# hal0zer0/openwurli

Measured on AMD Instinct MI355X. Metric: audio samples/s, 64-voice full chain (x real-time @48 kHz = value / 48000), higher is better.
Workload: dtype f64

## Files before the change

openwurli_amd/csrc/host/host_pool.inc:

```
namespace {
void trem_groups_changed(ow_pool* p) {
    HIP_OK(hipMemcpyAsync(p->d_lead, p->h_lead, sizeof(uint32_t) * p->I, hipMemcpyHostToDevice, p->stream));
    p->lead_list_valid = false;
    p->split_e0 = p->split_ne = -1;
}
void trem_split_at_range(ow_pool* p, int e0, int ne) {
    const uint32_t I = (uint32_t)p->I, lo = (uint32_t)e0, hi = (uint32_t)(e0 + ne);
    if (ne >= (int)I || (p->split_e0 == e0 && p->split_ne == ne)) return;
    const uint32_t NONE = 0xFFFFFFFFu;
    bool straddle = false;
    std::fill(p->grp_in.begin(), p->grp_in.end(), NONE);
    std::fill(p->grp_out.begin(), p->grp_out.end(), NONE);
    for (uint32_t e = 0; e < I; ++e) {
        const uint32_t x = p->h_lead[e];
        uint32_t& slot = (e >= lo && e < hi) ? p->grp_in[x] : p->grp_out[x];
        if (slot == NONE) slot = e;
    }
    size_t n_copy = 0;
    for (uint32_t x = 0; x < I; ++x) {
        if (p->grp_in[x] == NONE || p->grp_out[x] == NONE) continue;
        straddle = true;
        const bool x_inside = x >= lo && x < hi;
        const uint32_t fresh = x_inside ? p->grp_out[x] : p->grp_in[x];
        p->h_copy[n_copy] = x; p->h_copy[I + n_copy] = fresh; ++n_copy;
// ... 390 lines not shown
    return own_osc || hit ? p->rb_cur : -1;
}

struct Packed { bool any_dirty = false; size_t n_ops = 0; uint32_t n_act = 0; bool any_main = false, any_steal = false; };
static Packed pack_args_and_ops(ow_pool* p, const Block& b) {
    const int e0 = b.e0, ne = b.ne;
    Packed r;
    const bool untouched = b.whole && !__atomic_load_n(&p->dirty_any, __ATOMIC_RELAXED) && !p->args_stale && p->any_cache_valid;
    if (b.whole) __atomic_store_n(&p->dirty_any, (uint8_t)0, __ATOMIC_RELAXED);
    size_t n_dirty = 0;
    if (!untouched) for (int k = 0; k < ne; ++k) n_dirty += p->dirty[e0 + k];
    size_t T = (n_dirty >= 4096) ? std::min<size_t>(effective_cpus(), 32) : 1;
    const int per = (int)((ne + T - 1) / T);
    size_t cnt[OW_MAX_SLICES + 1] = {0};
    uint8_t dirty_t[OW_MAX_SLICES] = {0};
    auto count_slice = [&](size_t t) {
        size_t c = 0; uint8_t d = 0;
        const int k1 = std::min(ne, (int)(t + 1) * per);
        for (int k = (int)t * per; k < k1; ++k) {
            if (!p->dirty[e0 + k]) continue;
            d = 1;
            c += p->engines[e0 + k]->ops.size();
        }
        cnt[t + 1] = c; dirty_t[t] = d;
    };
    if (!untouched) Workers::get().each(T, count_slice);
    for (size_t t = 0; t < T; ++t) { r.any_dirty = r.any_dirty || dirty_t[t]; cnt[t + 1] += cnt[t]; }
    r.n_ops = cnt[T];
    ensure_ops_capacity(p, r.n_ops);
    if (r.any_dirty || p->args_stale) {
        auto pack_slice = [&](size_t t) {
            size_t op_pos = cnt[t];
            const int k1 = std::min(ne, (int)(t + 1) * per);
            for (int k = (int)t * per; k < k1; ++k) {
                OwEngineArgs& a = p->h_args[e0 + k];
                if (!p->dirty[e0 + k]) {
                    if (a.op_count || a.set_flags) { a.op_count = 0; a.set_flags = 0; }
                    continue;
                }
                ow_engine* en = p->engines[e0 + k].get();
                a.main_mask = en->vm->main_mask; a.steal_mask = en->vm->steal_mask;
                a.noise_on = en->noise_on ? 1u : 0u; a.thermal_gain = en->thermal_gain;
                a.pa_flags = en->rail_sag ? 1u : 0u;
                a.op_begin = (uint32_t)op_pos;
                a.op_count = (uint32_t)en->ops.size();
                if (!en->ops.empty()) std::memcpy(p->h_ops + op_pos, en->ops.data(), sizeof(OwOp) * en->ops.size());
                if (const uint32_t nd = en->vm->n_dev_ops) {
                    if (!en->ops.empty()) {
                        const uint32_t room = OW_VM_OPS_MAX - nd, nh = (uint32_t)std::min<size_t>(en->ops.size(), room);
                        if (nh < en->ops.size()) {
                            const uint64_t lost = g_ops_dropped.fetch_add(en->ops.size() - nh) + (en->ops.size() - nh);
                            if (lost == en->ops.size() - nh)
                                std::fprintf(stderr, "openwurli-hip: engine %zu: %zu queued slot ops do not fit behind a device-side MIDI burst (OW_MIDI_APPLY_EARLY=0) and are dropped\n",
                                             (size_t)(e0 + k), en->ops.size() - nh);
                        }
                        std::lock_guard<std::mutex> lk(p->op_tails_mu);
                        p->op_tails.push_back({(uint32_t)op_pos, (uint32_t)((e0 + k) * OW_VM_OPS_MAX) + nd, nh});
                        a.op_count = nd + nh;
                    } else a.op_count = nd;
                    a.op_begin = 0x80000000u | (uint32_t)((e0 + k) * OW_VM_OPS_MAX);
                    en->vm->n_dev_ops = 0;
                    if (!p->vm_host_dirty) p->vm_host_dirty = 1;
                }
                op_pos += en->ops.size();
                if (!en->ops.empty()) { en->ops.clear(); __atomic_fetch_sub(&p->host_ops_any, 1u, __ATOMIC_RELAXED); }
                a.set_flags = 0;
                if (en->depth.pending) { a.set_flags |= 1u; a.depth_target = en->depth.pending_value; en->depth.pending = false; }
                if (en->spk.pending)   { a.set_flags |= 2u; a.spk_target = en->spk.pending_value;     en->spk.pending = false; }
                if (en->volume.pending){ a.set_flags |= 4u; a.vol_target = en->volume.pending_value;  en->volume.pending = false; }
                p->dirty[e0 + k] = 0;
            }
        };
        Workers::get().each(T, pack_slice);
    }
    r.any_main = p->any_main_c; r.any_steal = p->any_steal_c;
    if (!untouched) {
        const size_t TA = ne >= 16384 ? std::min<size_t>(effective_cpus(), 32) : 1;
        const int per_a = (int)((ne + TA - 1) / TA);
        uint32_t act_n[OW_MAX_SLICES] = {0};
        uint8_t any_m[OW_MAX_SLICES] = {0}, any_s[OW_MAX_SLICES] = {0};
        auto scan_slice = [&](size_t t) {
            const int k0 = (int)t * per_a, k1 = std::min(ne, (int)(t + 1) * per_a);
            uint32_t n = 0; uint8_t m = 0, sl = 0;
            uint32_t* dst = p->h_op_engines + k0;
            for (int k = k0; k < k1; ++k) {
                const OwEngineArgs& a = p->h_args[e0 + k];
                m |= a.main_mask != 0; sl |= a.steal_mask != 0;
                if (a.op_count) dst[n++] = (uint32_t)(e0 + k);
            }
            act_n[t] = n; any_m[t] = m; any_s[t] = sl;
        };
        Workers::get().each(TA, scan_slice);
        r.any_main = false; r.any_steal = false;
        for (size_t t = 0; t < TA; ++t) {
            r.any_main |= any_m[t] != 0; r.any_steal |= any_s[t] != 0;
            if (act_n[t] && r.n_act != (uint32_t)(t * per_a)) std::memmove(p->h_op_engines + r.n_act, p->h_op_engines + t * per_a, sizeof(uint32_t) * act_n[t]);
            r.n_act += act_n[t];
        }
        if (b.whole) { p->any_main_c = r.any_main; p->any_steal_c = r.any_steal; p->any_cache_valid = true; }
    }
    return r;
}

static void upload_and_apply_ops(ow_pool* p, const Block& b, const Packed& pk) {
    const int e0 = b.e0, ne = b.ne;
    hipStream_t st = p->stream;
    if (pk.any_dirty || p->args_stale) {
        HIP_OK(hipMemcpyAsync(p->d_args + e0, p->h_args + e0, sizeof(OwEngineArgs) * ne, hipMemcpyHostToDevice, st));
        p->args_stale = pk.any_dirty;
    }
    HIP_OK(hipMemsetAsync(p->d_eout + e0, 0, sizeof(OwEngineOut) * ne, st));
    if (p->profiling) HIP_OK(hipEventRecord(p->ev[0], st));
    if (pk.n_ops || p->dev_ops_pending) {
        if (pk.n_ops) HIP_OK(hipMemcpyAsync(p->d_ops, p->h_ops, sizeof(OwOp) * pk.n_ops, hipMemcpyHostToDevice, st));
        for (const ow_pool::OpTail& t : p->op_tails)
            HIP_OK(hipMemcpyAsync(p->d_ops_fix + t.dst, p->d_ops + t.src, sizeof(OwOp) * t.n, hipMemcpyDeviceToDevice, st));
        p->op_tails.clear();
        if (pk.n_act) {
            HIP_OK(hipMemcpyAsync(p->d_op_engines, p->h_op_engines, sizeof(uint32_t) * pk.n_act, hipMemcpyHostToDevice, st));
            owdev::k_apply_ops<<<dim3(pk.n_act), dim3(64), 0, st>>>(p->dK, p->d_nt, p->d_vrec, p->d_args, p->d_ops, p->d_op_engines, p->d_ops_fix);
        }
        if (b.whole) p->dev_ops_pending = false;
    }
    if (p->profiling) HIP_OK(hipEventRecord(p->ev[1], st));
}

static bool launch_voices(ow_pool* p, const Block& b) {
    const int I = (int)p->I, L = b.L, Lcap = (int)p->Lcap;
    hipStream_t s = p->stream;
    const unsigned bs = p->vl_steady.n_blocks, bg = p->vl_general.n_blocks, bt = p->vl_steal.n_blocks, ba = p->vl_attack.n_blocks;
    if (ba) owdev::k_voice_steady<false, 1><<<dim3(ba), dim3(64), 0, s>>>(p->dK, p->d_vrec, p->vl_attack.d, p->d_sum, p->d_eout, I, L, Lcap, nullptr);
    if (bs) {
        if (p->sw.voice_skew && p->skew_next)
            owdev::k_voice_steady<true><<<dim3(bs), dim3(64), 0, s>>>(p->dK, p->d_vrec, p->vl_steady.d, p->d_sum, p->d_eout, I, L, Lcap, p->d_skew_seen);
        else
            owdev::k_voice_steady<false><<<dim3(bs), dim3(64), 0, s>>>(p->dK, p->d_vrec, p->vl_steady.d, p->d_sum, p->d_eout, I, L, Lcap, p->d_skew_seen);
    }
    if (bg) {
        const bool rel = p->sw.voice_release && !p->sw.force_general;
        if (rel) owdev::k_voice_steady<false, 3><<<dim3(bg), dim3(64), 0, s>>>(p->dK, p->d_vrec, p->vl_general.d, p->d_sum, p->d_eout, I, L, Lcap, nullptr);
        owdev::k_voice<<<dim3(bg), dim3(64), 0, s>>>(p->dK, p->d_vrec, p->vl_general.d, p->d_sum, p->d_eout, I, L, Lcap, rel ? 4 : 0);
    }
    if (bt) {
        if (p->sw.voice_steal) owdev::k_voice_steady<false, 2><<<dim3(bt), dim3(64), 0, s>>>(p->dK, p->d_vrec, p->vl_steal.d, p->d_sum, p->d_eout, I, L, Lcap, nullptr);
        owdev::k_voice<<<dim3(bt), dim3(64), 0, s>>>(p->dK, p->d_vrec, p->vl_steal.d, p->d_sum, p->d_eout, I, L, Lcap, p->sw.voice_steal ? 5 : 1);
    }
    return bs != 0;
}

static bool launch_chain(ow_pool* p, const Block& b, ChainKernel kernel) {
    const int I = (int)p->I, L = b.L, Lcap = (int)p->Lcap, e0 = b.e0, ne = b.ne;
    hipStream_t s = p->stream;
    const owdev::OwTremSrc& tsrc = b.tsrc;
    const dim3 per8((ne + 7) / 8), per32((ne + 31) / 32), per64((ne + 63) / 64);
    const int generic = p->sw.mel_generic ? 1 : 0;
    switch (kernel) {
    case CHAIN_NONE: break;
    case CHAIN_ROW_OS_8: owdev::k_chain_row<true, 8><<<per8, dim3(320), 0, s>>>(p->dK, p->d_cs, p->d_args, p->d_eout, p->d_sum, tsrc, p->d_pre, p->d_out, I, L, Lcap, L, e0, ne); break;
    case CHAIN_ROW_OS_16: owdev::k_chain_row<true, 16><<<per8, dim3(320), 0, s>>>(p->dK, p->d_cs, p->d_args, p->d_eout, p->d_sum, tsrc, p->d_pre, p->d_out, I, L, Lcap, L, e0, ne); break;
    case CHAIN_ROW_8: owdev::k_chain_row<false, 8><<<per8, dim3(320), 0, s>>>(p->dK, p->d_cs, p->d_args, p->d_eout, p->d_sum, tsrc, p->d_pre, p->d_out, I, L, Lcap, L, e0, ne); break;
    case CHAIN_ROW_16: owdev::k_chain_row<false, 16><<<per8, dim3(320), 0, s>>>(p->dK, p->d_cs, p->d_args, p->d_eout, p->d_sum, tsrc, p->d_pre, p->d_out, I, L, Lcap, L, e0, ne); break;
    case CHAIN_FUSED_OS: owdev::k_chain_fused<true><<<per8, dim3(128), 0, s>>>(p->dK, p->d_cs, p->d_args, p->d_eout, p->d_sum, tsrc, p->d_pre, p->d_out, I, L, Lcap, L, e0, ne); break;
    case CHAIN_FUSED: owdev::k_chain_fused<false><<<per8, dim3(128), 0, s>>>(p->dK, p->d_cs, p->d_args, p->d_eout, p->d_sum, tsrc, p->d_pre, p->d_out, I, L, Lcap, L, e0, ne); break;
    case CHAIN_STREAM:
        owdev::k_chain_stream<<<per32, dim3(64), 0, s>>>(p->dK, p->d_cs, p->d_args, p->d_eout, p->d_sum, tsrc, p->d_pre, p->d_out, I, L, Lcap, L, e0, ne, b.out_direct, b.out_stride);
        return b.out_direct != nullptr;
    case PREAMP_MEL_ENG:
        owdev::k_preamp_mel_eng<<<per64, dim3(64), 0, s>>>(p->dK, p->d_cs, p->d_mel_settled, p->d_args, p->d_eout, p->d_sum, tsrc, p->d_pre, p->d_noise, I, L, Lcap, e0, ne, generic, p->d_mel_lu, p->mel_lu_ld);
        break;
    case PREAMP_MEL_COL:
        owdev::k_preamp_mel_col<<<per32, dim3(64), 0, s>>>(p->dK, p->d_cs, p->d_mel_settled, p->d_args, p->d_eout, p->d_sum, tsrc, p->d_pre, p->d_noise, I, L, Lcap, e0, ne, generic, p->d_mel_lu, p->mel_lu_ld);
        break;
    case PREAMP_MEL_LIT:
        owdev::k_preamp_mel_lit<<<per32, dim3(64), 0, s>>>(p->dK, p->d_cs, p->d_mel_settled, p->d_args, p->d_eout, p->d_sum, tsrc, p->d_pre, p->d_noise, I, L, Lcap, e0, ne, generic, p->d_mel_lu);
        break;
    case PREAMP_MEL: owdev::k_preamp_mel<<<per32, dim3(64), 0, s>>>(p->dK, p->d_cs, p->d_mel_settled, p->d_args, p->d_eout, p->d_sum, tsrc, p->d_pre, p->d_noise, I, L, Lcap, e0, ne); break;
    case PREAMP_WIDE: owdev::k_preamp_wide<<<per8, dim3(64), 0, s>>>(p->dK, p->d_cs, p->d_args, p->d_eout, p->d_sum, tsrc, p->d_pre, I, L, Lcap, e0, ne); break;
    case PREAMP_PAIR: owdev::k_preamp_pair<<<per64, dim3(64), 0, s>>>(p->dK, p->d_cs, p->d_args, p->d_eout, p->d_sum, tsrc, p->d_pre, I, L, Lcap, e0, ne); break;
    case PREAMP_LANE: owdev::k_preamp<<<per32, dim3(64), 0, s>>>(p->dK, p->d_cs, p->d_args, p->d_eout, p->d_sum, tsrc, p->d_pre, I, L, Lcap, e0, ne); break;
    }
    return false;
}

static bool launch_output_stage(ow_pool* p, const Block& b, PostKernel kernel) {
    const int I = (int)p->I, L = b.L, e0 = b.e0, ne = b.ne;
    hipStream_t s = p->stream;
    switch (kernel) {
    case POST_NONE: return false;
    case POST_MPA: {
        const bool ordered = p->sw.pa_sort != 0 && ne > power_amp_resident_engines(p);
        if (ordered) {
            const uint32_t total = (uint32_t)b.n_os;
            HIP_OK(hipMemsetAsync(p->d_pa_hist, 0, sizeof(uint32_t) * PA_ORDER_CLASSES, s));
            owdev::k_pa_order_hist<<<dim3((ne + 255) / 256), dim3(256), 0, s>>>(p->d_pa_demand, e0, ne, total, p->d_pa_hist);
            owdev::k_pa_order_scan<<<dim3(1), dim3(PA_ORDER_CLASSES), 0, s>>>(p->d_pa_hist);
            owdev::k_pa_order_scatter<<<dim3((ne + 255) / 256), dim3(256), 0, s>>>(p->d_pa_demand, e0, ne, total, p->d_pa_hist, p->d_pa_order);
        }
        owdev::k_post_mpa<<<dim3((ne + PA_EPB - 1) / PA_EPB), dim3(PA_WPB * 64), 0, s>>>(p->dK, p->dPa, p->d_pa_settled, p->d_cs, p->d_pa, p->d_args, p->d_eout, p->d_pre, p->d_out,
                                                                                     p->d_pa_tap, I, L, L, e0, ne, ordered ? p->d_pa_order : nullptr, p->d_pa_demand);
        return false;
    }
    case POST_PAIR: owdev::k_post<false, true><<<dim3((ne + 63) / 64), dim3(64), 0, s>>>(p->dK, p->d_cs, p->d_args, p->d_eout, p->d_pre, p->d_out, I, L, L, e0, ne, b.out_direct, b.out_stride); break;
    case POST_OS: owdev::k_post<true><<<dim3((ne + 31) / 32), dim3(64), 0, s>>>(p->dK, p->d_cs, p->d_args, p->d_eout, p->d_pre, p->d_out, I, L, L, e0, ne, b.out_direct, b.out_stride); break;
    case POST_BASE: owdev::k_post<false><<<dim3((ne + 63) / 64), dim3(64), 0, s>>>(p->dK, p->d_cs, p->d_args, p->d_eout, p->d_pre, p->d_out, I, L, L, e0, ne, b.out_direct, b.out_stride); break;
    }
    return b.out_direct != nullptr;
}

static void deliver_rows(ow_pool* p, const Block& b) {
    const float* src = p->d_out + (size_t)b.e0 * b.len;
    if (b.out_stride == b.len) HIP_OK(hipMemcpyAsync(b.out_host, src, sizeof(float) * b.len * (size_t)b.ne, hipMemcpyDeviceToHost, p->stream));
    else HIP_OK(hipMemcpy2DAsync(b.out_host, b.out_stride * sizeof(float), src, b.len * sizeof(float), b.len * sizeof(float), (size_t)b.ne, hipMemcpyDeviceToHost, p->stream));
}

static void finish_block(ow_pool* p, const Block& b, bool steady_launched) {
    const int e0 = b.e0, ne = b.ne, n_os = b.n_os;
    hipStream_t st = p->stream;
    if (b.chain && p->traj) {
        if (b.whole) p->trem_clock += n_os;
        else {
            for (int k = 0; k < ne; ++k) if (p->h_birth[e0 + k] != OW_OFF_TRAJ) { p->h_birth[e0 + k] -= n_os; p->min_birth = std::min(p->min_birth, p->h_birth[e0 + k]); }
            owdev::k_trem_birth_shift<<<dim3((ne + 255) / 256), dim3(256), 0, st>>>(p->d_birth, e0, ne, -(long long)n_os);
        }
    }
    p->last_n_os = n_os;
    HIP_OK(hipGetLastError());
    if (steady_launched) {
        HIP_OK(hipMemcpyAsync(p->h_skew_seen, p->d_skew_seen, sizeof(uint32_t), hipMemcpyDeviceToHost, st));
        p->skew_pending = true;
    }
    if (eout_attention(p, ne)) {
        if (p->attn_resync) {
            std::memcpy(p->h_prev_tr, p->transient.data(), p->I);
            HIP_OK(hipMemcpyAsync(p->d_prev_tr, p->h_prev_tr, p->I, hipMemcpyHostToDevice, st));
            p->attn_resync = false;
        }
        owdev::k_eout_attention<<<dim3((ne + 255) / 256), dim3(256), 0, st>>>(p->d_eout, p->d_args, p->d_prev_tr, e0, ne, p->d_attn);
        HIP_OK(hipGetLastError());
        HIP_OK(hipMemcpyAsync(p->h_attn, p->d_attn, sizeof(uint64_t) * ((ne + 63) / 64), hipMemcpyDeviceToHost, st));
        p->attn_pending = true;
    } else {
        HIP_OK(hipMemcpyAsync(p->h_eout + e0, p->d_eout + e0, sizeof(OwEngineOut) * ne, hipMemcpyDeviceToHost, st));
        p->attn_pending = false;
    }
}

void render_range(ow_pool* p, int e0, int ne, size_t len, bool with_voices, float* out_host = nullptr, size_t out_stride = 0) {
    if (len > p->Lcap) { HIP_OK(hipStreamSynchronize(p->stream)); alloc_stream_buffers(p, len); }
    p->out_ld = len;
    hipStream_t st = p->stream;
    auto profile_mark = [&](int i) { if (p->profiling) HIP_OK(hipEventRecord(p->ev_stage[i], st)); };
    vm_wait_download(p);
    Block b;
    b.e0 = e0; b.ne = ne; b.len = len; b.L = (int)len; b.n_os = b.L * (p->hc.oversample ? 2 : 1);
    b.whole = e0 == 0 && ne == (int)p->I;
    b.chain = !p->voices_only;
    b.out_host = out_host; b.out_stride = out_stride;
    b.tsrc = owdev::OwTremSrc{nullptr, p->d_lead, nullptr, p->d_birth};
    const hipEvent_t traj_ready = b.chain && p->traj ? traj_cover_block(p, b) : nullptr;
    const int trem_half = trem_block(p, b);
    const Packed pk = pack_args_and_ops(p, b);
    upload_and_apply_ops(p, b, pk);
    const bool voices = with_voices && (pk.any_main || pk.any_steal);
    if (voices) {
        if (!p->lists_valid || pk.any_dirty || p->lists_e0 != e0 || p->lists_ne != ne) build_voice_lists(p, e0, ne);
        p->lists_valid = !pk.any_dirty;
        if (p->vl_steady.n_blocks) HIP_OK(hipMemsetAsync(p->d_skew_seen, 0, sizeof(uint32_t), st));
    }
    if (out_host && p->sw.out_direct != 0 && out_stride >= len && ne > 0)
        b.out_direct = (float*)host_block_device_ptr(out_host, sizeof(float) * ((size_t)(ne - 1) * out_stride + len));
    profile_mark(0);
    const bool steady_launched = voices && launch_voices(p, b);
    profile_mark(1);
    if (trem_half >= 0) HIP_OK(hipStreamWaitEvent(st, p->ev_trem[trem_half], 0));
    if (traj_ready) HIP_OK(hipStreamWaitEvent(st, traj_ready, 0));
    profile_mark(2);
    const ChainKernel chain = !b.chain ? CHAIN_NONE
        : choose_chain(p->sw, (int)p->hc.preamp_kind, p->power_amp_kind, p->hc.oversample != 0, p->hc.ml_sparse_ok != 0, ne, b.L, b.out_direct != nullptr);
    bool delivered = launch_chain(p, b, chain);
    profile_mark(3);
    delivered |= launch_output_stage(p, b, choose_post(p->sw, p->power_amp_kind, p->hc.oversample != 0, ne, chain));
    profile_mark(4);
    if (out_host && ne > 0 && !delivered) deliver_rows(p, b);
    finish_block(p, b, steady_launched);
}

void engine_steal_countdown(ow_engine* en, uint32_t l32) {
    OwVm& v = *en->vm;
    if (!v.steal_mask) return;
    vm_host_changed(en);
    for (uint64_t m = v.steal_mask; m; m &= m - 1) {
        const int s = __builtin_ctzll(m);
        v.steal_fade[s] = v.steal_fade[s] > l32 ? v.steal_fade[s] - l32 : 0u;
        if (v.steal_fade[s] == 0) { v.has_steal &= ~(1ull << s); en->sync_masks(s); }
    }
}
void engine_post_render(ow_engine* en, uint32_t l32, const OwEngineOut& o, bool steal_counted = false) {
    OwVm& v = *en->vm;
    vm_host_changed(en);
    if (!steal_counted) engine_steal_countdown(en, l32);
    if (o.sum_nonfinite) {
        en->nan_guard_fires += 1;
        for (int s = 0; s < OW_MAX_VOICES; ++s) {
            const uint64_t b = 1ull << s;
            if ((o.bad_main >> s) & 1ull) { en->set_state(s, OW_VOICE_FREE); v.has_voice &= ~b; }
            if ((o.bad_steal >> s) & 1ull) { v.has_steal &= ~b; v.steal_fade[s] = 0; }
            en->sync_masks(s);
        }
    }
    if (o.out_nonfinite) en->output_nan_resets += 1;
    for (uint64_t m = o.silent_mask & v.main_mask; m; m &= m - 1) {
        const int s = __builtin_ctzll(m);
        if (en->state_of(s) != OW_VOICE_FREE && ((v.has_voice >> s) & 1ull)) { en->set_state(s, OW_VOICE_FREE); v.has_voice &= ~(1ull << s); en->sync_masks(s); }
    }
}

void engine_guard_second_pass_result(ow_engine* en, const OwEngineOut& o) {
    OwVm& v = *en->vm;
    vm_host_changed(en);
    for (int s = 0; s < OW_MAX_VOICES; ++s) {
        const uint64_t b = 1ull << s;
        bool touched = false;
        if ((o.bad_main >> s) & 1ull) { en->set_state(s, OW_VOICE_FREE); v.has_voice &= ~b; touched = true; }
        if ((o.bad_steal >> s) & 1ull) { v.has_steal &= ~b; v.steal_fade[s] = 0; touched = true; }
        if (touched) en->sync_masks(s);
    }
    for (uint64_t m = o.silent_mask & v.main_mask; m; m &= m - 1) {
        const int s = __builtin_ctzll(m);
        if (en->state_of(s) != OW_VOICE_FREE && ((v.has_voice >> s) & 1ull)) { en->set_state(s, OW_VOICE_FREE); v.has_voice &= ~(1ull << s); en->sync_masks(s); }
    }
}
void guard_second_pass(ow_pool* p, const uint32_t* engs, size_t n_eng, size_t len) {
    hipStream_t st = p->stream;
    uint32_t nm = 0, ns = 0;
    for (size_t i = 0; i < n_eng; ++i) {
        const ow_engine* en = p->engines[engs[i]].get();
        auto put = [&](uint32_t* a, uint32_t& n, uint64_t mask) {
            if (!mask) return;
            for (uint64_t m = mask; m; m &= m - 1) a[n++] = (engs[i] << 6) | (uint32_t)__builtin_ctzll(m);
            while (n & 63u) a[n++] = 0xFFFFFFFFu;
        };
        put(p->vl_general.h, nm, en->vm->main_mask);
        put(p->vl_steal.h, ns, en->vm->steal_mask);
    }
    p->lists_valid = false;
    p->vl_general.sig_valid = false; p->vl_steal.sig_valid = false;
    const unsigned nb = (unsigned)((n_eng + 255) / 256);
    HIP_OK(hipMemcpyAsync(p->d_op_engines, engs, sizeof(uint32_t) * n_eng, hipMemcpyHostToDevice, st));
    owdev::k_eout_clear_list<<<dim3(nb), dim3(256), 0, st>>>(p->d_eout, p->d_op_engines, (int)n_eng);
    const int I = (int)p->I, L = (int)len, Lcap = (int)p->Lcap;
    if (nm) {
        HIP_OK(hipMemcpyAsync(p->vl_general.d, p->vl_general.h, sizeof(uint32_t) * nm, hipMemcpyHostToDevice, st));
        owdev::k_voice<<<dim3(nm / 64), dim3(64), 0, st>>>(p->dK, p->d_vrec, p->vl_general.d, p->d_sum, p->d_eout, I, L, Lcap, 2);
    }
    if (ns) {
// ... 283 lines not shown
```

openwurli_amd/csrc/ow_kernels.h:

```cpp
#pragma once
#include "ow_vm.h"
#include "ow_chain_dev.h"

namespace owdev {

#define OW_DATA_DECL __device__ const
#define OW_GEN_DATA_REINCLUDE
#include "../../data/ow_gen_data.h"
#undef OW_GEN_DATA_REINCLUDE
#undef OW_DATA_DECL

struct OwEngineOut {
    uint64_t silent_mask;
    uint64_t bad_main;
    uint64_t bad_steal;
    uint32_t sum_nonfinite;
    uint32_t out_nonfinite;
    uint32_t transient;
    uint32_t pad;
};

__device__ inline void mlp_raw_scalar(double in0, double in1, double raw[11]) {
    double h1[16], h2[16];
    for (int i = 0; i < 16; ++i) {
        double sum = MLP_B1[i];
        sum += MLP_W1[i][0] * in0;
        sum += MLP_W1[i][1] * in1;
        h1[i] = sum > 0.0 ? sum : 0.0;
    }
    for (int i = 0; i < 16; ++i) {
        double sum = MLP_B2[i];
        for (int j = 0; j < 16; ++j) sum += MLP_W2[i][j] * h1[j];
        h2[i] = sum > 0.0 ? sum : 0.0;
    }
    for (int i = 0; i < 11; ++i) {
        double sum = MLP_B3[i];
        for (int j = 0; j < 16; ++j) sum += MLP_W3[i][j] * h2[j];
        raw[i] = sum * MLP_TARGET_STDS[i] + MLP_TARGET_MEANS[i];
    }
}

#ifndef OW_APPLY_OPS_ATTR
#define OW_APPLY_OPS_ATTR __attribute__((amdgpu_waves_per_eu(2, 2)))
#endif
__device__ inline void mlp_raw_mfma(double* __restrict__ h, double in0, double in1, double raw[11]);

__global__ __launch_bounds__(64) OW_APPLY_OPS_ATTR void k_apply_ops(const OwConsts* __restrict__ K, const double* __restrict__ nt, double* __restrict__ vrec,
                                                  const OwEngineArgs* __restrict__ args, const OwOp* __restrict__ ops_packed,
                                                  const uint32_t* __restrict__ engines, const OwOp* __restrict__ ops_fixed = nullptr,
                                                  const OwVm* __restrict__ vm = nullptr, int e_base = 0) {
    __shared__ double h[64 * 17];
    const int e = vm ? e_base + (int)blockIdx.x : (int)engines[blockIdx.x];
    const int lane = threadIdx.x;
    OwEngineArgs a;
    if (vm) { a.op_count = vm[e].n_dev_ops; a.op_begin = 0x80000000u | (uint32_t)(e * OW_VM_OPS_MAX); }
    else a = args[e];
    if (a.op_count == 0) return;
    const OwOp* __restrict__ ops = (a.op_begin & 0x80000000u) ? ops_fixed : ops_packed;
    a.op_begin &= 0x7FFFFFFFu;
    double* main_rec = vrec + ((size_t)e * 2 + 0) * OW_VREC_DOUBLES + lane;
    double* steal_rec = vrec + ((size_t)e * 2 + 1) * OW_VREC_DOUBLES + lane;
    constexpr int OPS_TILES = 8;
    uint64_t mine[OPS_TILES];
    const bool tiled = a.op_count <= 64u * OPS_TILES;
    if (tiled) {
#pragma unroll
        for (int t = 0; t < OPS_TILES; ++t) {
            mine[t] = 0ull;
            if ((uint32_t)t * 64u < a.op_count) {
                const uint32_t idx = (uint32_t)t * 64u + (uint32_t)lane;
                const int sl = idx < a.op_count ? (int)ops[a.op_begin + idx].slot : -1;
                for (int v = 0; v < 64; ++v) {
                    const uint64_t m = __ballot(sl == v);
                    if (lane == v) mine[t] = m;
                }
            }
        }
    }
    uint32_t cursor = 0;
    for (;;) {
        asm volatile("" : "+v"(main_rec), "+v"(steal_rec));
        OwOp op;
        op.type = 0;
        if (tiled) {
            bool got = false;
#pragma unroll
            for (int t = 0; t < OPS_TILES; ++t) {
                if (!got && mine[t]) {
                    const int b = __builtin_ctzll(mine[t]);
                    mine[t] &= mine[t] - 1ull;
                    op = ops[a.op_begin + (uint32_t)t * 64u + (uint32_t)b];
                    got = true;
                }
            }
        } else {
            while (cursor < a.op_count) {
                const OwOp cand = ops[a.op_begin + cursor];
                ++cursor;
                if (cand.slot == lane) { op = cand; break; }
            }
        }
        if (!__any(op.type != 0)) break;
        const bool is_on = op.type == OP_NOTE_ON;
        if (__any(is_on)) {
            const double midi = is_on ? (double)op.note : 60.0;
            const double in0 = clampd((midi - 21.0) / (108.0 - 21.0), 0.0, 1.0);
            const double in1 = is_on ? clampd(op.velocity, 0.0, 1.0) : 0.0;
            double raw[11];
            mlp_raw_mfma(h, in0, in1, raw);
            if (is_on) {
                const MlpOut corr = mlp_finish((int)op.note, raw, op.mlp != 0);
                note_on_lane(main_rec, nt, K, (int)op.note, op.velocity, op.seed, corr);
            }
        }
        if (op.type == OP_DAMPER) {
            start_damper_lane(main_rec, K);
        } else if (op.type == OP_SET_DS) {
            main_rec[VF_DS * 64] = op.velocity;
        } else if (op.type == OP_MOVE_STEAL) {
            constexpr int CP = 16;
            for (int f0 = 0; f0 < VF_COUNT; f0 += CP) {
                double t[CP];
#pragma unroll
                for (int k = 0; k < CP; ++k) t[k] = f0 + k < VF_COUNT ? main_rec[(f0 + k) * 64] : 0.0;
#pragma unroll
                for (int k = 0; k < CP; ++k) if (f0 + k < VF_COUNT) steal_rec[(f0 + k) * 64] = t[k];
            }
            steal_rec[VF_STEAL * 64] = bitsd((uint64_t)op.seed | ((uint64_t)op.seed << 32));
        }
    }
}

#ifndef OW_VOICE_GENERAL_ATTR
#define OW_VOICE_GENERAL_ATTR __attribute__((amdgpu_waves_per_eu(2, 2)))
#endif
#define OW_VCHUNK 24
#define OW_NO_VOICE 0xFFFFFFFFu

struct VoiceLanes {
    int e, slot;
    bool active;
    uint64_t seg_end;
    int nvalid;
};
OW_DEV VoiceLanes voice_lanes(const uint32_t* __restrict__ entries, int* __restrict__ eng_l) {
    const int lane = threadIdx.x;
    const uint32_t ent = entries[(size_t)blockIdx.x * 64 + lane];
    VoiceLanes w;
    w.active = ent != OW_NO_VOICE;
    w.e = w.active ? (int)(ent >> 6) : -1;
    w.slot = (int)(ent & 63u);
    eng_l[lane] = w.e;
    const int e_next = __shfl_down(w.e, 1);
    w.seg_end = __ballot(w.active && (lane == 63 || e_next != w.e));
    w.nvalid = __popcll(__ballot(w.active));
// ... 812 lines not shown
        rbuf[(size_t)i * I + e] = trem_cell_r(t, P, K, M + z);
    }
    trem_store(t, P, cs, I, e);
}
__global__ __launch_bounds__(64) void k_tremolo(const OwConsts* __restrict__ K, double* __restrict__ cs, double* __restrict__ rbuf, int I, int n_os,
                                                const uint32_t* __restrict__ leaders, int n_lead) {
    __shared__ TremMats M;
    __shared__ TremPark P;
    tremolo_body(K, cs, rbuf, I, n_os, leaders, n_lead, &M, &P);
}
__global__ __launch_bounds__(64) void k_tremolo_lfo(const OwConsts* __restrict__ K, double* __restrict__ cs, double* __restrict__ rbuf, int I, long long n_os,
                                                    const uint32_t* __restrict__ leaders, int n_lead, long long n_extra) {
    const int idx = blockIdx.x * 64 + threadIdx.x;
    if (idx >= n_lead) return;
    const int e = (int)leaders[idx];
    double phase = CSF(CS_T_V), env = CSF(CS_T_ENV), r_ldr = CSF(CS_T_RLDR);
    const double inc = K->lfo_phase_inc, two_pi = 2.0 * 3.14159265358979323846264338327950288;
    const long long n = n_os + n_extra * idx;
    for (long long i = 0; i < n; ++i) {
        const double lfo = sin(phase);
        phase += inc;
        if (phase >= two_pi) phase -= two_pi;
        const double led = lfo > 0.0 ? lfo : 0.0;
        const double coeff = led > env ? K->ldr_attack : K->ldr_release;
        env = led + coeff * (env - led);
        const double drive = clampd(env, 0.0, 1.0);
        if (drive < 1e-6) r_ldr = 1000000.0;
        else r_ldr = exp(K->ln_r_max + K->ln_min_minus_max * pow(drive, 0.9));
        if (rbuf) rbuf[(size_t)i * I + e] = r_ldr;
    }
    CSF(CS_T_V) = phase; CSF(CS_T_ENV) = env; CSF(CS_T_RLDR) = r_ldr;
}

#define OW_PCHUNK 64
__global__ __launch_bounds__(64) void k_preamp(const OwConsts* __restrict__ K, double* __restrict__ cs, const OwEngineArgs* __restrict__ args,
                                               const OwEngineOut* __restrict__ eout, const double* __restrict__ sum, const OwTremSrc tsrc,
                                               double* __restrict__ pre, int I, int L, int Lcap, int e0, int ne) {
    __shared__ double tile[32 * (OW_PCHUNK + 1)];
    const int lane = threadIdx.x;
    const int el = lane & 31, role = lane >> 5;
    const int eb = e0 + blockIdx.x * 32;
    const int e = eb + el;
    const bool valid = e < e0 + ne;
    const int ec = valid ? e : (e0 + ne - 1);
    const int osr = K->oversample ? 2 : 1;

    DkSt st;
    double ua[3], ub[3];
    double r_ldr, g_ldr, g_prev;
    Smoother sd;
    {
        const int e = ec;
        smoother_load(sd, cs, I, e, CS_SM_DEPTH);
        if (args[e].set_flags & 1u) sd.retarget(args[e].depth_target, K->ramp_samples);
        dk_load(st, cs, I, e, role ? CS_P_SHADOW : CS_P_MAIN);
        for (int i = 0; i < 3; ++i) { ua[i] = CSF(CS_OS_UA + i); ub[i] = CSF(CS_OS_UB + i); }
        r_ldr = CSF(CS_P_RLDR); g_ldr = CSF(CS_P_GLDR); g_prev = CSF(CS_P_GPREV);
        const uint64_t fl = dbits(CSF(CS_FLAGS));
        if (fl & 1ull) {
            dk_dc_reset(K, r_ldr, st);
            g_ldr = 1.0 / r_ldr; g_prev = g_ldr;
            for (int i = 0; i < 3; ++i) { ua[i] = 0.0; ub[i] = 0.0; }
        }
    }
    uint32_t nan_resets = 0;
    double sh_depth = __longlong_as_double(0x7FF8000000000000LL), sh_top = 0.0, sh_lower = 0.0;
    int rowflag = 0;
    {
        const int er = eb + el;
        if (er < e0 + ne && !eout[er].sum_nonfinite) rowflag = (args[er].main_mask ? 1 : 0) | (args[er].steal_mask ? 2 : 0);
    }
    const int e_last = e0 + ne - 1;
    const TremCol tcol = trem_col(tsrc, I, ec);
    double rn[2];
    rn[0] = trem_col_at(tcol, 0u);
    rn[1] = osr == 2 ? trem_col_at(tcol, 1u) : 0.0;
    for (int base = 0; base < L; base += OW_PCHUNK) {
        const int cn = min(OW_PCHUNK, L - base);
        const int col = base + min(lane, cn - 1);
#pragma unroll 8
        for (int r = 0; r < 32; ++r) {
            const int er = min(eb + r, e_last);
            const int fl = __builtin_amdgcn_readlane(rowflag, r);
            const double a = sum[((size_t)0 * I + er) * Lcap + col];
            const double b = sum[((size_t)1 * I + er) * Lcap + col];
            double x = (fl & 1) ? a : 0.0;
            x = (fl & 2) ? x + b : x;
            tile[r * (OW_PCHUNK + 1) + lane] = x;
        }
        __syncthreads();
        for (int n = 0; n < cn; ++n) {
            const double x = tile[el * (OW_PCHUNK + 1) + n];
            const double rc[2] = {rn[0], rn[1]};
            {
                const uint32_t nx = (uint32_t)(min(base + n + 1, L - 1) * osr);
                rn[0] = trem_col_at(tcol, nx);
                if (osr == 2) rn[1] = trem_col_at(tcol, nx + 1u);
            }
            const double depth = clampd(sd.next(), 0.0, 1.0);
            if (__builtin_amdgcn_ballot_w64(!(depth == sh_depth)) != 0ull) {
                sh_depth = depth;
                const double r_upper = 50000.0 * (1.0 - depth);
                sh_lower = 50000.0 * depth;
                sh_top = r_upper > 0.0 ? ow_div(r_upper * 18000.0, r_upper + 18000.0) : 0.0;
            }
            double in[2];
            if (osr == 2) {
                const double a = allpass3(OW_OS_A0, OW_OS_A1, OW_OS_A2, ua, x);
                const double b = allpass3(OW_OS_B0, OW_OS_B1, OW_OS_B2, ub, x);
                in[0] = role ? 0.0 : a;
                in[1] = role ? 0.0 : b;
            } else {
                in[0] = role ? 0.0 : x;
                in[1] = 0.0;
            }
            for (int j = 0; j < osr; ++j) {
                const size_t idx = (size_t)((base + n) * osr + j);
                const double branch = 680.0 + rc[j];
                const double low = sh_lower > 0.0 ? ow_div(sh_lower * branch, sh_lower + branch) : 0.0;
                const double r_new = fmax(sh_top + low, 1000.0);
                if (fabs(r_new - r_ldr) > 0.01) { r_ldr = r_new; g_ldr = ow_div(1.0, r_new); }
                const double o = dk_step(st, in[j], g_ldr, g_prev, K);
                g_prev = g_ldr;
                const double other = xor32_t(o);
                double result = role ? (other - o) : (o - other);
                if (!isfinite(result)) {
                    dk_dc_reset(K, r_ldr, st);
                    g_ldr = 1.0 / r_ldr; g_prev = g_ldr;
                    result = 0.0;
                    nan_resets += 1u;
                }
                if (valid && role == 0) pre[idx * I + e] = result;
            }
        }
        __syncthreads();
    }
    if (valid) {
        dk_store(st, cs, I, e, role ? CS_P_SHADOW : CS_P_MAIN);
        if (role == 0) {
            for (int i = 0; i < 3; ++i) { CSF(CS_OS_UA + i) = ua[i]; CSF(CS_OS_UB + i) = ub[i]; }
            CSF(CS_P_RLDR) = r_ldr; CSF(CS_P_GLDR) = g_ldr; CSF(CS_P_GPREV) = g_prev;
            smoother_store(sd, cs, I, e, CS_SM_DEPTH);
            const uint64_t fl = dbits(CSF(CS_FLAGS));
            if (fl & 1ull) CSF(CS_FLAGS) = bitsd(fl & ~1ull);
            if (nan_resets) {
                const uint64_t d = dbits(CSF(CS_DIAG));
                CSF(CS_DIAG) = bitsd((d & 0xFFFFFFFFull) | ((uint64_t)((uint32_t)(d >> 32) + nan_resets) << 32));
            }
        }
    }
}

#define OW_PPCHUNK 32
__global__ __launch_bounds__(64) __attribute__((amdgpu_waves_per_eu(2, 2)))
void k_preamp_pair(const OwConsts* __restrict__ K, double* __restrict__ cs, const OwEngineArgs* __restrict__ args,
                   const OwEngineOut* __restrict__ eout, const double* __restrict__ sum, const OwTremSrc tsrc,
                   double* __restrict__ pre, int I, int L, int Lcap, int e0, int ne) {
    __shared__ double tile[64 * (OW_PPCHUNK + 1)];
    const int lane = threadIdx.x;
    const int eb = e0 + blockIdx.x * 64;
    const int e = eb + lane;
    const bool valid = e < e0 + ne;
    const int ec = valid ? e : (e0 + ne - 1);
    const int osr = K->oversample ? 2 : 1;

    DkSt sm, ss;
    double ua[3], ub[3];
    double r_ldr, g_ldr, g_prev;
    Smoother sd;
    {
        const int e = ec;
        smoother_load(sd, cs, I, e, CS_SM_DEPTH);
        if (args[e].set_flags & 1u) sd.retarget(args[e].depth_target, K->ramp_samples);
        dk_load(sm, cs, I, e, CS_P_MAIN);
        dk_load(ss, cs, I, e, CS_P_SHADOW);
        for (int i = 0; i < 3; ++i) { ua[i] = CSF(CS_OS_UA + i); ub[i] = CSF(CS_OS_UB + i); }
        r_ldr = CSF(CS_P_RLDR); g_ldr = CSF(CS_P_GLDR); g_prev = CSF(CS_P_GPREV);
        const uint64_t fl = dbits(CSF(CS_FLAGS));
        if (fl & 1ull) {
            dk_dc_reset(K, r_ldr, sm);
            ss = sm;
            g_ldr = 1.0 / r_ldr; g_prev = g_ldr;
            for (int i = 0; i < 3; ++i) { ua[i] = 0.0; ub[i] = 0.0; }
        }
    }
    DkPairRes R;
    dk_pair_res_load(R, K);
    uint32_t nan_resets = 0;
    double sh_depth = __longlong_as_double(0x7FF8000000000000LL), sh_top = 0.0, sh_lower = 0.0;
    int rowflag = 0;
    if (valid && !eout[e].sum_nonfinite) rowflag = (args[e].main_mask ? 1 : 0) | (args[e].steal_mask ? 2 : 0);
    const int e_last = e0 + ne - 1;
    const int half = lane >> 5;
    const TremCol tcol = trem_col(tsrc, I, ec);
    double rn[2];
    rn[0] = trem_col_at(tcol, 0u);
    rn[1] = osr == 2 ? trem_col_at(tcol, 1u) : 0.0;
    for (int base = 0; base < L; base += OW_PPCHUNK) {
        const int cn = min(OW_PPCHUNK, L - base);
        const int col = base + min(lane & 31, cn - 1);
#pragma unroll 8
        for (int r = 0; r < 32; ++r) {
            const int row = r + 32 * half;
            const int er = min(eb + row, e_last);
            const int fl_lo = __builtin_amdgcn_readlane(rowflag, r), fl_hi = __builtin_amdgcn_readlane(rowflag, r + 32);
            const int fl = half ? fl_hi : fl_lo;
            const double a = sum[((size_t)0 * I + er) * Lcap + col];
            const double b = sum[((size_t)1 * I + er) * Lcap + col];
            double x = (fl & 1) ? a : 0.0;
            x = (fl & 2) ? x + b : x;
            tile[row * (OW_PPCHUNK + 1) + (lane & 31)] = x;
        }
        __syncthreads();
        for (int n = 0; n < cn; ++n) {
            const double x = tile[lane * (OW_PPCHUNK + 1) + n];
            const double rc[2] = {rn[0], rn[1]};
            {
                const uint32_t nx = (uint32_t)(min(base + n + 1, L - 1) * osr);
                rn[0] = trem_col_at(tcol, nx);
                if (osr == 2) rn[1] = trem_col_at(tcol, nx + 1u);
            }
            const double depth = clampd(sd.next(), 0.0, 1.0);
            if (__builtin_amdgcn_ballot_w64(!(depth == sh_depth)) != 0ull) {
                sh_depth = depth;
                const double r_upper = 50000.0 * (1.0 - depth);
                sh_lower = 50000.0 * depth;
                sh_top = r_upper > 0.0 ? ow_div(r_upper * 18000.0, r_upper + 18000.0) : 0.0;
            }
            double in[2];
            if (osr == 2) {
                in[0] = allpass3(OW_OS_A0, OW_OS_A1, OW_OS_A2, ua, x);
                in[1] = allpass3(OW_OS_B0, OW_OS_B1, OW_OS_B2, ub, x);
            } else {
                in[0] = x;
                in[1] = 0.0;
            }
            for (int j = 0; j < osr; ++j) {
                const size_t idx = (size_t)((base + n) * osr + j);
                const double branch = 680.0 + (j ? rc[1] : rc[0]);
                const double low = sh_lower > 0.0 ? ow_div(sh_lower * branch, sh_lower + branch) : 0.0;
                const double r_new = fmax(sh_top + low, 1000.0);
                if (fabs(r_new - r_ldr) > 0.01) { r_ldr = r_new; g_ldr = ow_div(1.0, r_new); }
                double om, os;
                dk_step_pair(sm, ss, j ? in[1] : in[0], 0.0, g_ldr, g_prev, K, R, om, os);
                g_prev = g_ldr;
                double result = om - os;
                if (!isfinite(result)) {
                    dk_dc_reset(K, r_ldr, sm);
                    ss = sm;
                    g_ldr = 1.0 / r_ldr; g_prev = g_ldr;
                    result = 0.0;
                    nan_resets += 1u;
                }
                if (valid) pre[idx * I + e] = result;
            }
        }
        __syncthreads();
    }
    if (valid) {
        dk_store(sm, cs, I, e, CS_P_MAIN);
        dk_store(ss, cs, I, e, CS_P_SHADOW);
        for (int i = 0; i < 3; ++i) { CSF(CS_OS_UA + i) = ua[i]; CSF(CS_OS_UB + i) = ub[i]; }
        CSF(CS_P_RLDR) = r_ldr; CSF(CS_P_GLDR) = g_ldr; CSF(CS_P_GPREV) = g_prev;
        smoother_store(sd, cs, I, e, CS_SM_DEPTH);
        const uint64_t fl = dbits(CSF(CS_FLAGS));
        if (fl & 1ull) CSF(CS_FLAGS) = bitsd(fl & ~1ull);
        if (nan_resets) {
            const uint64_t d = dbits(CSF(CS_DIAG));
            CSF(CS_DIAG) = bitsd((d & 0xFFFFFFFFull) | ((uint64_t)((uint32_t)(d >> 32) + nan_resets) << 32));
        }
    }
}

#define OW_OCHUNK 64
template <bool SPLIT, bool PAIR = false>
__global__ __launch_bounds__(64) void k_post(const OwConsts* __restrict__ K, double* __restrict__ cs, const OwEngineArgs* __restrict__ args,
                                             OwEngineOut* __restrict__ eout, const double* __restrict__ pre, float* __restrict__ out, int I, int L,
                                             int Lcap, int e0, int ne, float* __restrict__ out2 = nullptr, size_t ld2 = 0) {
    constexpr int NROWS = SPLIT ? 32 : 64;
    __shared__ float tile[NROWS * (OW_OCHUNK + 1)];
    const int lane = threadIdx.x;
    const int el = SPLIT ? (lane & 31) : lane;
    const int phase = SPLIT ? (lane >> 5) : 0;
    const int eb = e0 + blockIdx.x * NROWS;
    const int e_raw = eb + el;
    const bool valid = e_raw < e0 + ne;
    const int e = valid ? e_raw : (e0 + ne - 1);
    static_assert(!(SPLIT && PAIR), "PAIR is the lane = engine form of the oversampled chain");
    const int osr = (SPLIT || PAIR) ? 2 : 1;
    const double sr = K->sr;
    const double thermal_alpha = K->spk_thermal_alpha;

    double da[3], db[3], dd;
    for (int i = 0; i < 3; ++i) { da[i] = CSF(CS_OS_DA + i); db[i] = CSF(CS_OS_DB + i); }
    dd = CSF(CS_OS_DD);
    SpeakerSt sp;
    {
        double* hp = &sp.hpf.b0; double* lp = &sp.lpf.b0;
        for (int i = 0; i < 7; ++i) { hp[i] = CSF(CS_SPK_HPF + i); lp[i] = CSF(CS_SPK_LPF + i); }
        sp.character = CSF(CS_SPK_CHAR); sp.a2 = CSF(CS_SPK_A2); sp.a3 = CSF(CS_SPK_A3); sp.tc = CSF(CS_SPK_TC); sp.ts = CSF(CS_SPK_TS);
    }
    Smoother ss, sv;
    smoother_load(ss, cs, I, e, CS_SM_SPK);
    smoother_load(sv, cs, I, e, CS_SM_VOL);
    if (args[e].set_flags & 2u) ss.retarget(args[e].spk_target, K->ramp_samples);
    if (args[e].set_flags & 4u) sv.retarget(args[e].vol_target, K->ramp_samples);
    bool nan_fired = false;

    double pn = pre[(size_t)phase * I + e];
    double pn1 = PAIR ? pre[(size_t)I + e] : 0.0;
    for (int base = 0; base < L; base += OW_OCHUNK) {
        const int cn = min(OW_OCHUNK, L - base);
        for (int n = 0; n < cn; ++n) {
            const double pc = pn, pc1 = pn1;
            pn = pre[((size_t)min(base + n + 1, L - 1) * osr + phase) * I + e];
            if (PAIR) pn1 = pre[((size_t)min(base + n + 1, L - 1) * 2 + 1) * I + e];
            const double y = power_amp(pc * 0.25);
            double o;
            if (PAIR) {
                const double y1 = power_amp(pc1 * 0.25);
                const double a = allpass3(OW_OS_A0, OW_OS_A1, OW_OS_A2, da, y);
                const double b = allpass3(OW_OS_B0, OW_OS_B1, OW_OS_B2, db, y1);
                o = (a + dd) * 0.5;
                dd = b;
            } else if (SPLIT) {
                const double yo = xor32_t(y);
                const double y0 = phase ? yo : y, y1 = phase ? y : yo;
                const double a = allpass3(OW_OS_A0, OW_OS_A1, OW_OS_A2, da, y0);
                const double b = allpass3(OW_OS_B0, OW_OS_B1, OW_OS_B2, db, y1);
                o = (a + dd) * 0.5;
                dd = b;
            } else {
                o = y;
            }
            speaker_set_character(sp, ss.next(), sr);
            const double shaped = speaker_process(sp, o, thermal_alpha);
            const double post = shaped * 7.498942093324558 * sv.next();
            float f = (float)post;
            if (!isfinite(f)) {
                f = 0.0f;
                sp.hpf.s1 = sp.hpf.s2 = sp.lpf.s1 = sp.lpf.s2 = 0.0;
                sp.ts = 0.0;
                nan_fired = true;
            }
            if (phase == 0) tile[el * (OW_OCHUNK + 1) + n] = f;
        }
        __syncthreads();
        for (int r = 0; r < NROWS; ++r) {
            const int er = eb + r;
            if (er < e0 + ne && lane < cn) {
                const float f = tile[r * (OW_OCHUNK + 1) + lane];
                out[(size_t)er * Lcap + base + lane] = f;
                if (out2) out2[(size_t)(er - e0) * ld2 + base + lane] = f;
            }
        }
        __syncthreads();
    }
    if (!valid || phase != 0) return;
    if (nan_fired) {
        for (int i = 0; i < 3; ++i) { da[i] = 0.0; db[i] = 0.0; }
        dd = 0.0;
        CSF(CS_FLAGS) = bitsd(dbits(CSF(CS_FLAGS)) | 1ull);
        eout[e].out_nonfinite = 1u;
    }
    for (int i = 0; i < 3; ++i) { CSF(CS_OS_DA + i) = da[i]; CSF(CS_OS_DB + i) = db[i]; }
    CSF(CS_OS_DD) = dd;
    {
        const double* hp = &sp.hpf.b0; const double* lp = &sp.lpf.b0;
        for (int i = 0; i < 7; ++i) { CSF(CS_SPK_HPF + i) = hp[i]; CSF(CS_SPK_LPF + i) = lp[i]; }
        CSF(CS_SPK_CHAR) = sp.character; CSF(CS_SPK_A2) = sp.a2; CSF(CS_SPK_A3) = sp.a3; CSF(CS_SPK_TC) = sp.tc; CSF(CS_SPK_TS) = sp.ts;
    }
    smoother_store(ss, cs, I, e, CS_SM_SPK);
    smoother_store(sv, cs, I, e, CS_SM_VOL);
}

}
```

Before: 3.783 billion.

## Pack eight waves per block and balance SIMD-paired waves with priority turns

The pair preamp and pair post kernels now run eight independent 64-lane waves per workgroup instead of one. Each wave works on its own engines with its own LDS tile, and block-wide barriers are replaced by wave-local syncs. A new WaveTurns helper finds the wave sharing the same SIMD through the hardware SIMD id register and raises s_setprio on whichever wave of the pair is behind, so the two progress in step. This aims to improve latency hiding and issue interleaving between co-resident waves, at the cost of per-sample LDS atomic traffic and a larger launch granularity that can leave CUs idle when the engine count is small.

```diff
diff --git a/openwurli_amd/csrc/host/host_pool.inc b/openwurli_amd/csrc/host/host_pool.inc
--- a/openwurli_amd/csrc/host/host_pool.inc
+++ b/openwurli_amd/csrc/host/host_pool.inc
@@ -566,7 +566,7 @@
     const int I = (int)p->I, L = b.L, Lcap = (int)p->Lcap, e0 = b.e0, ne = b.ne;
     hipStream_t s = p->stream;
     const owdev::OwTremSrc& tsrc = b.tsrc;
-    const dim3 per8((ne + 7) / 8), per32((ne + 31) / 32), per64((ne + 63) / 64);
+    const dim3 per8((ne + 7) / 8), per32((ne + 31) / 32), per64((ne + 63) / 64), per512((ne + 511) / 512);
     const int generic = p->sw.mel_generic ? 1 : 0;
     switch (kernel) {
     case CHAIN_NONE: break;
@@ -590,7 +590,7 @@
         break;
     case PREAMP_MEL: owdev::k_preamp_mel<<<per32, dim3(64), 0, s>>>(p->dK, p->d_cs, p->d_mel_settled, p->d_args, p->d_eout, p->d_sum, tsrc, p->d_pre, p->d_noise, I, L, Lcap, e0, ne); break;
     case PREAMP_WIDE: owdev::k_preamp_wide<<<per8, dim3(64), 0, s>>>(p->dK, p->d_cs, p->d_args, p->d_eout, p->d_sum, tsrc, p->d_pre, I, L, Lcap, e0, ne); break;
-    case PREAMP_PAIR: owdev::k_preamp_pair<<<per64, dim3(64), 0, s>>>(p->dK, p->d_cs, p->d_args, p->d_eout, p->d_sum, tsrc, p->d_pre, I, L, Lcap, e0, ne); break;
+    case PREAMP_PAIR: owdev::k_preamp_pair<<<per512, dim3(512), 0, s>>>(p->dK, p->d_cs, p->d_args, p->d_eout, p->d_sum, tsrc, p->d_pre, I, L, Lcap, e0, ne); break;
     case PREAMP_LANE: owdev::k_preamp<<<per32, dim3(64), 0, s>>>(p->dK, p->d_cs, p->d_args, p->d_eout, p->d_sum, tsrc, p->d_pre, I, L, Lcap, e0, ne); break;
     }
     return false;
@@ -614,7 +614,7 @@
                                                                                      p->d_pa_tap, I, L, L, e0, ne, ordered ? p->d_pa_order : nullptr, p->d_pa_demand);
         return false;
     }
-    case POST_PAIR: owdev::k_post<false, true><<<dim3((ne + 63) / 64), dim3(64), 0, s>>>(p->dK, p->d_cs, p->d_args, p->d_eout, p->d_pre, p->d_out, I, L, L, e0, ne, b.out_direct, b.out_stride); break;
+    case POST_PAIR: owdev::k_post<false, true><<<dim3((ne + 511) / 512), dim3(512), 0, s>>>(p->dK, p->d_cs, p->d_args, p->d_eout, p->d_pre, p->d_out, I, L, L, e0, ne, b.out_direct, b.out_stride); break;
     case POST_OS: owdev::k_post<true><<<dim3((ne + 31) / 32), dim3(64), 0, s>>>(p->dK, p->d_cs, p->d_args, p->d_eout, p->d_pre, p->d_out, I, L, L, e0, ne, b.out_direct, b.out_stride); break;
     case POST_BASE: owdev::k_post<false><<<dim3((ne + 63) / 64), dim3(64), 0, s>>>(p->dK, p->d_cs, p->d_args, p->d_eout, p->d_pre, p->d_out, I, L, L, e0, ne, b.out_direct, b.out_stride); break;
     }
diff --git a/openwurli_amd/csrc/ow_kernels.h b/openwurli_amd/csrc/ow_kernels.h
--- a/openwurli_amd/csrc/ow_kernels.h
+++ b/openwurli_amd/csrc/ow_kernels.h
@@ -1,6 +1,7 @@
 #pragma once
 #include "ow_vm.h"
 #include "ow_chain_dev.h"
+#include "ow_wave_turns.h"
 
 namespace owdev {
 
@@ -1119,13 +1120,19 @@
 }
 
 #define OW_PPCHUNK 32
-__global__ __launch_bounds__(64) __attribute__((amdgpu_waves_per_eu(2, 2)))
+__global__ __launch_bounds__(64 * OW_TURN_WAVES) __attribute__((amdgpu_waves_per_eu(2, 2)))
 void k_preamp_pair(const OwConsts* __restrict__ K, double* __restrict__ cs, const OwEngineArgs* __restrict__ args,
                    const OwEngineOut* __restrict__ eout, const double* __restrict__ sum, const OwTremSrc tsrc,
                    double* __restrict__ pre, int I, int L, int Lcap, int e0, int ne) {
-    __shared__ double tile[64 * (OW_PPCHUNK + 1)];
-    const int lane = threadIdx.x;
-    const int eb = e0 + blockIdx.x * 64;
+    __shared__ double tiles[OW_TURN_WAVES * 64 * (OW_PPCHUNK + 1)];
+    __shared__ uint32_t turn_words[OW_TURN_LDS_WORDS];
+    WaveTurns turns;
+    turns.init(turn_words);
+    const int wave = __builtin_amdgcn_readfirstlane((int)(threadIdx.x >> 6));
+    double* const tile = tiles + wave * (64 * (OW_PPCHUNK + 1));
+    const int lane = threadIdx.x & 63;
+    const int eb = e0 + (blockIdx.x * OW_TURN_WAVES + wave) * 64;
+    if (eb >= e0 + ne) { turns.finish(); return; }
     const int e = eb + lane;
     const bool valid = e < e0 + ne;
     const int ec = valid ? e : (e0 + ne - 1);
@@ -1178,8 +1185,9 @@
             x = (fl & 2) ? x + b : x;
             tile[row * (OW_PPCHUNK + 1) + (lane & 31)] = x;
         }
-        __syncthreads();
+        wave_sync();
         for (int n = 0; n < cn; ++n) {
+            turns.tick((uint32_t)(base + n));
             const double x = tile[lane * (OW_PPCHUNK + 1) + n];
             const double rc[2] = {rn[0], rn[1]};
             {
@@ -1222,8 +1230,9 @@
                 if (valid) pre[idx * I + e] = result;
             }
         }
-        __syncthreads();
-    }
+        wave_sync();
+    }
+    turns.finish();
     if (valid) {
         dk_store(sm, cs, I, e, CS_P_MAIN);
         dk_store(ss, cs, I, e, CS_P_SHADOW);
@@ -1241,15 +1250,28 @@
 
 #define OW_OCHUNK 64
 template <bool SPLIT, bool PAIR = false>
-__global__ __launch_bounds__(64) void k_post(const OwConsts* __restrict__ K, double* __restrict__ cs, const OwEngineArgs* __restrict__ args,
-                                             OwEngineOut* __restrict__ eout, const double* __restrict__ pre, float* __restrict__ out, int I, int L,
-                                             int Lcap, int e0, int ne, float* __restrict__ out2 = nullptr, size_t ld2 = 0) {
+__global__ __launch_bounds__(64 * (PAIR ? OW_TURN_WAVES : 1))
+void k_post(const OwConsts* __restrict__ K, double* __restrict__ cs, const OwEngineArgs* __restrict__ args,
+            OwEngineOut* __restrict__ eout, const double* __restrict__ pre, float* __restrict__ out, int I, int L,
+            int Lcap, int e0, int ne, float* __restrict__ out2 = nullptr, size_t ld2 = 0) {
     constexpr int NROWS = SPLIT ? 32 : 64;
-    __shared__ float tile[NROWS * (OW_OCHUNK + 1)];
-    const int lane = threadIdx.x;
+    constexpr int W = PAIR ? OW_TURN_WAVES : 1;
+    __shared__ float tiles[W * NROWS * (OW_OCHUNK + 1)];
+    __shared__ uint32_t turn_words[PAIR ? OW_TURN_LDS_WORDS : 1];
+    WaveTurns turns;
+    int wave = 0;
+    if constexpr (PAIR) {
+        turns.init(turn_words);
+        wave = __builtin_amdgcn_readfirstlane((int)(threadIdx.x >> 6));
+    }
+    float* const tile = tiles + wave * (NROWS * (OW_OCHUNK + 1));
+    const int lane = PAIR ? (threadIdx.x & 63) : threadIdx.x;
     const int el = SPLIT ? (lane & 31) : lane;
     const int phase = SPLIT ? (lane >> 5) : 0;
-    const int eb = e0 + blockIdx.x * NROWS;
+    const int eb = e0 + (blockIdx.x * W + wave) * NROWS;
+    if constexpr (PAIR) {
+        if (eb >= e0 + ne) { turns.finish(); return; }
+    }
     const int e_raw = eb + el;
     const bool valid = e_raw < e0 + ne;
     const int e = valid ? e_raw : (e0 + ne - 1);
@@ -1279,6 +1301,7 @@
     for (int base = 0; base < L; base += OW_OCHUNK) {
         const int cn = min(OW_OCHUNK, L - base);
         for (int n = 0; n < cn; ++n) {
+            if constexpr (PAIR) turns.tick((uint32_t)(base + n));
             const double pc = pn, pc1 = pn1;
             pn = pre[((size_t)min(base + n + 1, L - 1) * osr + phase) * I + e];
             if (PAIR) pn1 = pre[((size_t)min(base + n + 1, L - 1) * 2 + 1) * I + e];
@@ -1312,7 +1335,7 @@
             }
             if (phase == 0) tile[el * (OW_OCHUNK + 1) + n] = f;
         }
-        __syncthreads();
+        if constexpr (PAIR) wave_sync(); else __syncthreads();
         for (int r = 0; r < NROWS; ++r) {
             const int er = eb + r;
             if (er < e0 + ne && lane < cn) {
@@ -1321,8 +1344,9 @@
                 if (out2) out2[(size_t)(er - e0) * ld2 + base + lane] = f;
             }
         }
-        __syncthreads();
-    }
+        if constexpr (PAIR) wave_sync(); else __syncthreads();
+    }
+    if constexpr (PAIR) turns.finish();
     if (!valid || phase != 0) return;
     if (nan_fired) {
         for (int i = 0; i < 3; ++i) { da[i] = 0.0; db[i] = 0.0; }
diff --git a/openwurli_amd/csrc/ow_wave_turns.h b/openwurli_amd/csrc/ow_wave_turns.h
--- /dev/null
+++ b/openwurli_amd/csrc/ow_wave_turns.h
@@ -0,0 +1,62 @@
+#pragma once
+#include <hip/hip_runtime.h>
+#include <stdint.h>
+
+namespace owdev {
+
+#define OW_TURN_WAVES 8
+#define OW_TURN_LDS_WORDS (2 * OW_TURN_WAVES)
+#define OW_TURN_FINISHED 0xFFFFFFFFu
+#define OW_HWREG_SIMD_ID (4 | (4 << 6) | ((2 - 1) << 11))
+
+__device__ __forceinline__ void wave_sync() {
+    __builtin_amdgcn_fence(__ATOMIC_RELEASE, "wavefront");
+    __builtin_amdgcn_wave_barrier();
+    __builtin_amdgcn_fence(__ATOMIC_ACQUIRE, "wavefront");
+}
+
+struct WaveTurns {
+    uint32_t* mine;
+    const uint32_t* theirs;
+    int prio;
+
+    static __device__ __forceinline__ void put(uint32_t* p, uint32_t v) { __hip_atomic_store(p, v, __ATOMIC_RELAXED, __HIP_MEMORY_SCOPE_WORKGROUP); }
+    static __device__ __forceinline__ uint32_t get(const uint32_t* p) {
+        return (uint32_t)__builtin_amdgcn_readfirstlane((int)__hip_atomic_load(p, __ATOMIC_RELAXED, __HIP_MEMORY_SCOPE_WORKGROUP));
+    }
+
+    __device__ __forceinline__ void init(uint32_t* lds, bool enable = true) {
+        const int w = __builtin_amdgcn_readfirstlane((int)(threadIdx.x >> 6));
+        const uint32_t simd = __builtin_amdgcn_s_getreg(OW_HWREG_SIMD_ID);
+        mine = lds + OW_TURN_WAVES + w;
+        put(lds + w, simd);
+        put(mine, 0u);
+        __syncthreads();
+        int partner = w, n = 0;
+        for (int i = 0; i < OW_TURN_WAVES; ++i) {
+            const uint32_t s = get(lds + i);
+            if (i != w && s == simd) { partner = i; ++n; }
+        }
+        if (!enable || n != 1) partner = w;
+        theirs = lds + OW_TURN_WAVES + __builtin_amdgcn_readfirstlane(partner);
+        prio = 0;
+    }
+
+    __device__ __forceinline__ void tick(uint32_t done) {
+        put(mine, done);
+        const uint32_t other = get(theirs);
+        const uint32_t me = (uint32_t)__builtin_amdgcn_readfirstlane((int)done);
+        if (me < other) {
+            if (prio == 0) { __builtin_amdgcn_s_setprio(1); prio = 1; }
+        } else if (me > other) {
+            if (prio != 0) { __builtin_amdgcn_s_setprio(0); prio = 0; }
+        }
+    }
+
+    __device__ __forceinline__ void finish() {
+        put(mine, OW_TURN_FINISHED);
+        if (prio != 0) { __builtin_amdgcn_s_setprio(0); prio = 0; }
+    }
+};
+
+}
```

New measurement: 3.944 billion, median of 6. +4.3%, better.
